# weleen/AGRL.pytorch

Hardware: AMD Instinct MI355X
Metric: frames/sec (fwd+GCN+distmat), MARS seq_len=8 (higher is better)
Workload: dtype fp16; 1 GPU; MARS seq_len=8 bs=32/GPU fp16 fwd+distmat (BASELINE configs[1]): 256x128 frames, VMGN ResNet50x2-branch + 2 graph layers, cosine distmat vs resident 12180 x 4096 gallery; global_batch=32, seq_len=8, gallery_rows_per_gpu=12180, parallelism=dp1, hip_graph=False, ranks=1, devices_visible=1, library=libagrl_hip.so, clip_batches_rotated=3, clip_bytes_rotated=301989888

## Files before the change

### agrl.pytorch_amd/csrc/agrl_common.h

```cpp
#pragma once
#include <hip/hip_runtime.h>
#include <math.h>
#include <stdint.h>
#include <stdio.h>
#include <stdarg.h>

#include "../../include/agrl_hip.h"

#define AGRL_WAVE 64

#ifndef AGRL_LP_F16
#define AGRL_LP_F16 1
#endif
constexpr bool kLpF16 = AGRL_LP_F16 != 0;
typedef unsigned short lp16_t;
typedef __attribute__((ext_vector_type(8))) __bf16 bf16x8_t;
typedef __attribute__((ext_vector_type(8))) _Float16 f16x8_t;
typedef __attribute__((ext_vector_type(4))) float f32x4_t;

void agrl_set_error(const char* fmt, ...);

#define AGRL_CHECK_ARG(cond, ...)       \
    do {                                \
        if (!(cond)) {                  \
            agrl_set_error(__VA_ARGS__); \
            return 1;                   \
        }                               \
    } while (0)

#define AGRL_CHECK_LAUNCH(name)                                                   \
    do {                                                                          \
        hipError_t e__ = hipGetLastError();                                       \
        if (e__ != hipSuccess) {                                                  \
            agrl_set_error("%s: launch failed: %s", name, hipGetErrorString(e__)); \
            return 2;                                                             \
        }                                                                         \
    } while (0)

static inline bool agrl_is_pow2(float v) {
    int e = 0;
    return v > 0.f && v <= 3.4e38f && frexpf(v, &e) == 0.5f;
}
#define AGRL_CHECK_POW2(value, who, name) \
    AGRL_CHECK_ARG(agrl_is_pow2(value), "%s: %s=%g is not a positive finite power of two", who, name, (double)(value))

__attribute__((visibility("hidden"))) int agrl_cu_count();

typedef __attribute__((address_space(3))) void lds_void_t;
typedef __attribute__((address_space(1))) const void gbl_void_t;

__host__ __device__ inline float lp16_to_f32(lp16_t v) {
    if constexpr (kLpF16) {
        return (float)__builtin_bit_cast(_Float16, v);
    } else {
        return __builtin_bit_cast(float, ((uint32_t)v) << 16);
    }
}

__host__ __device__ inline lp16_t f32_to_lp16(float f) {
    if constexpr (kLpF16) {
        return __builtin_bit_cast(unsigned short, (_Float16)f);
    } else {
#if defined(__HIP_DEVICE_COMPILE__)
        const __bf16 h = (__bf16)f;
        return __builtin_bit_cast(unsigned short, h);
#else
        uint32_t u = __builtin_bit_cast(uint32_t, f);
        if ((u & 0x7fffffffu) > 0x7f800000u) return (lp16_t)((u >> 16) | 0x40);
        u += 0x7fffu + ((u >> 16) & 1u);
        return (lp16_t)(u >> 16);
#endif
    }
}

__device__ inline uint32_t pack_lp16x2(float lo, float hi) {
    if constexpr (kLpF16) {
        typedef __attribute__((ext_vector_type(2))) _Float16 f16x2_t;
        const f16x2_t v = {(_Float16)lo, (_Float16)hi};
        return __builtin_bit_cast(uint32_t, v);
    } else {
        typedef __attribute__((ext_vector_type(2))) __bf16 bf16x2_t;
        const bf16x2_t v = {(__bf16)lo, (__bf16)hi};
        return __builtin_bit_cast(uint32_t, v);
    }
}

__device__ inline uint32_t pack_bf16x2(float lo, float hi) {
    typedef __attribute__((ext_vector_type(2))) __bf16 bf16x2_t;
    const bf16x2_t v = {(__bf16)lo, (__bf16)hi};
    return __builtin_bit_cast(uint32_t, v);
}

__device__ inline void unpack_lp16x2(uint32_t w, float& lo, float& hi) {
    if constexpr (kLpF16) {
        typedef __attribute__((ext_vector_type(2))) _Float16 f16x2_t;
        const f16x2_t v = __builtin_bit_cast(f16x2_t, w);
        lo = (float)v[0];
        hi = (float)v[1];
    } else {
        lo = __uint_as_float(w << 16);
        hi = __uint_as_float(w & 0xffff0000u);
    }
}

template <typename TA, typename TB>
__device__ inline __attribute__((ext_vector_type(4))) float mfma_lp16_16x16x32(const TA& a, const TB& b, __attribute__((ext_vector_type(4))) float c) {
    static_assert(sizeof(TA) == 16 && sizeof(TB) == 16, "16-byte MFMA operands");
    if constexpr (kLpF16) {
        return __builtin_amdgcn_mfma_f32_16x16x32_f16(__builtin_bit_cast(f16x8_t, a), __builtin_bit_cast(f16x8_t, b), c, 0, 0, 0);
    } else {
        return __builtin_amdgcn_mfma_f32_16x16x32_bf16(__builtin_bit_cast(bf16x8_t, a), __builtin_bit_cast(bf16x8_t, b), c, 0, 0, 0);
    }
}

__device__ inline float relu_nan(float v) { return __builtin_elementwise_maximum(v, 0.f); }

__device__ inline float wave_sum(float v) {
#pragma unroll
    for (int off = 32; off > 0; off >>= 1) v += __shfl_xor(v, off, 64);
    return v;
}

__device__ inline float wave_max(float v) {
#pragma unroll
    for (int off = 32; off > 0; off >>= 1) v = fmaxf(v, __shfl_xor(v, off, 64));
    return v;
}

__device__ inline int wave_sum_i(int v) {
#pragma unroll
    for (int off = 32; off > 0; off >>= 1) v += __shfl_xor(v, off, 64);
    return v;
}

template <typename T>
struct DT;
template <>
struct DT<float> {
    static constexpr int code = AGRL_F32;
    static constexpr int epc = 4;
    __device__ static inline float ld(const float* p) { return *p; }
    __device__ static inline void st(float* p, float v) { *p = v; }
};
struct f32s_t {
    float v;
};
template <>
struct DT<f32s_t> {
    static constexpr int code = AGRL_F32X3;
    static constexpr int epc = 4;
};
struct f32h_t {
    float v;
};
template <>
struct DT<f32h_t> {
    static constexpr int code = AGRL_F32H3;
    static constexpr int epc = 4;
};
template <>
struct DT<lp16_t> {
    static constexpr int code = AGRL_LP16;
    static constexpr int epc = 8;
    __device__ static inline float ld(const lp16_t* p) { return lp16_to_f32(*p); }
    __device__ static inline void st(lp16_t* p, float v) { *p = f32_to_lp16(v); }
};

static inline int cdiv(int a, int b) { return (a + b - 1) / b; }

#define AGRL_OPT_UNSET (-2147483647 - 1)
struct AgrlOpts {
    int igemm_wide;
    int pool_persist;
    int conv3x3_wide, conv3x3_c64;
    int distmat_tiled;
    int topk_radix;
    int graph_linear_mmajor;
    int conv3x3_n128;
    int conv3x3_fat_pb;
    int conv3x3_half, conv3x3_half_stagger;
    int stem_split_lds;
    int stem_xcd_map;
    int distmat_tile_n;
    int split16_ns;
    int duo_persist;
    int igemm_dbg, conv3x3_dbg;
};
const AgrlOpts& agrl_opts();
inline bool agrl_opt_set(int v) { return v != AGRL_OPT_UNSET; }

#ifdef AGRL_ABLATE
#define AGRL_DBG_BITS(p) ((p).dbg)
#else
#define AGRL_DBG_BITS(p) 0
#endif
```

### agrl.pytorch_amd/csrc/common.hip

```cpp
#include "agrl_common.h"

static thread_local char g_err[512] = "";

void agrl_set_error(const char* fmt, ...) {
    va_list ap;
    va_start(ap, fmt);
    vsnprintf(g_err, sizeof(g_err), fmt, ap);
    va_end(ap);
}

extern "C" int agrl_version(void) { return 100; }
extern "C" const char* agrl_last_error(void) { return g_err; }

extern "C" int agrl_lp16_is_f16(void) { return kLpF16 ? 1 : 0; }

#include <atomic>

int agrl_cu_count() {
    constexpr int kMaxDev = 64;
    static std::atomic<int> cache[kMaxDev];
    int dev = 0;
    if (hipGetDevice(&dev) != hipSuccess) return 256;
    const bool slot = dev >= 0 && dev < kMaxDev;
    int n = slot ? cache[dev].load(std::memory_order_relaxed) : 0;
    if (n > 0) return n;
    if (hipDeviceGetAttribute(&n, hipDeviceAttributeMultiprocessorCount, dev) != hipSuccess || n <= 0) n = 256;
    if (slot) cache[dev].store(n, std::memory_order_relaxed);
    return n;
}

#include <stdlib.h>

static int opt_int(const char* name) {
    const char* e = getenv(name);
    return e ? atoi(e) : AGRL_OPT_UNSET;
}
static int opt_flag(const char* name) {
    const char* e = getenv(name);
    return e && !(e[0] == '0' && e[1] == 0) ? 1 : 0;
}
static AgrlOpts load_opts() {
    AgrlOpts o;
    o.igemm_wide = opt_int("AGRL_IGEMM_WIDE");
    o.pool_persist = opt_flag("AGRL_POOL_PERSIST");
    o.conv3x3_wide = opt_int("AGRL_CONV3X3_WIDE");
    o.conv3x3_c64 = opt_int("AGRL_CONV3X3_C64");
    o.distmat_tiled = opt_flag("AGRL_DISTMAT_TILED");
    o.topk_radix = opt_flag("AGRL_TOPK_RADIX");
    o.graph_linear_mmajor = opt_flag("AGRL_GRAPH_LINEAR_MMAJOR");
    o.conv3x3_n128 = opt_flag("AGRL_CONV3X3_N128");
    o.distmat_tile_n = opt_int("AGRL_DISTMAT_TILE_N");
    o.duo_persist = opt_int("AGRL_DUO_PERSIST");
    o.split16_ns = opt_int("AGRL_SPLIT16_NS");
    o.stem_xcd_map = opt_int("AGRL_STEM_XCD_MAP");
    o.stem_split_lds = opt_int("AGRL_STEM_SPLIT_LDS");
    o.conv3x3_fat_pb = opt_int("AGRL_CONV3X3_FAT_PB");
    o.conv3x3_half = opt_int("AGRL_CONV3X3_HALF");
    o.conv3x3_half_stagger = opt_int("AGRL_CONV3X3_HALF_STAGGER");
#ifdef AGRL_ABLATE
    o.igemm_dbg = agrl_opt_set(opt_int("AGRL_IGEMM_DBG")) ? opt_int("AGRL_IGEMM_DBG") : 0;
    o.conv3x3_dbg = agrl_opt_set(opt_int("AGRL_CONV3X3_DBG")) ? opt_int("AGRL_CONV3X3_DBG") : 0;
#else
    o.igemm_dbg = 0;
    o.conv3x3_dbg = 0;
#endif
    return o;
}
static AgrlOpts g_opts = load_opts();

const AgrlOpts& agrl_opts() { return g_opts; }
extern "C" int agrl_reload_options(void) {
    g_opts = load_opts();
    return 0;
}
extern "C" int agrl_built_with_ablation(void) {
#ifdef AGRL_ABLATE
    return 1;
#else
    return 0;
#endif
}
```

### agrl.pytorch_amd/csrc/stem_dev.h

```cpp
#pragma once
#include "agrl_common.h"
#include "frames_u8.h"

struct StemShape {
    int CH, CW;
    int PH, PW;
    int tiles_h, tiles_w;
    int grid;
};

static inline int stem_shape(const char* who, int N, int H, int W, int pt_h, int pt_w, StemShape* s) {
    AGRL_CHECK_ARG(N > 0 && H >= 7 && W >= 7, "%s: bad shape N=%d H=%d W=%d", who, N, H, W);
    s->CH = (H + 6 - 7) / 2 + 1, s->CW = (W + 6 - 7) / 2 + 1;
    s->PH = (s->CH + 2 - 3) / 2 + 1, s->PW = (s->CW + 2 - 3) / 2 + 1;
    s->tiles_h = cdiv(s->PH, pt_h), s->tiles_w = cdiv(s->PW, pt_w);
    const long long grid = (long long)N * s->tiles_h * s->tiles_w;
    AGRL_CHECK_ARG(grid < (1ll << 31), "%s: grid too large", who);
    s->grid = (int)grid;
    return 0;
}

namespace stem8 {
constexpr int PT = 8;
constexpr int CT = 2 * PT + 1;
constexpr int NPOS = CT * CT;
constexpr int NFRAG = (NPOS + 15) / 16;
constexpr int NWV = 8;
constexpr int NTH = 64 * NWV;
constexpr int FPW = (NFRAG + NWV - 1) / NWV;
constexpr int IT = 2 * (CT - 1) + 7;
constexpr int PWP = 40;
constexpr int PATCH_BYTES = IT * PWP * 8;
constexpr int NPASS = (IT * PWP + NTH - 1) / NTH;
constexpr int WROW_BYTES = 480;
constexpr int W_BYTES = 64 * WROW_BYTES;

struct Tile {
    int n, ph0, pw0, cr0, cc0;
};
__device__ __forceinline__ Tile tile_at(int T, int tiles_w, int tiles_hw) {
    Tile t;
    t.n = T / tiles_hw;
    const int trem = T - t.n * tiles_hw;
    t.ph0 = (trem / tiles_w) * PT, t.pw0 = (trem % tiles_w) * PT;
    t.cr0 = 2 * t.ph0 - 1, t.cc0 = 2 * t.pw0 - 1;
    return t;
}

template <typename TIN, typename... EX>
struct PatchPrefetch {
    static constexpr bool U8 = sizeof...(EX) != 0;
    uint32_t pb[U8 ? NPASS : 1][3];
    float pv[NPASS][3];

    __device__ __forceinline__ void load(const TIN* __restrict__ x, int H, int W, const Tile& t, EX... ex) {
        const int iy0 = 2 * t.cr0 - 3, ix0 = 2 * t.cc0 - 3;
        const TIN* xn = x + (size_t)t.n * 3 * H * W;
        int td = threadIdx.x;
        asm volatile("" : "+v"(td));
#pragma unroll
        for (int i = 0; i < NPASS; ++i) {
            const int e = td + NTH * i;
            const int py = e / PWP, px = e - py * PWP;
            const int iy = iy0 + py, ix = ix0 + px;
            if constexpr (U8) {
                const FramesU8 u8 = frames_u8_of(ex...);
                pb[i][0] = pb[i][1] = pb[i][2] = FRAMES_U8_PAD;
                if (e < IT * PWP && px < IT && (unsigned)iy < (unsigned)H && (unsigned)ix < (unsigned)W) {
                    const uint32_t o = (uint32_t)(iy * W + ix) * u8.pixel_stride;
                    pb[i][0] = xn[o];
                    pb[i][1] = xn[o + (uint32_t)u8.channel_stride];
                    pb[i][2] = xn[o + 2 * (uint32_t)u8.channel_stride];
                }
            } else {
                pv[i][0] = pv[i][1] = pv[i][2] = 0.f;
                if (e < IT * PWP && px < IT && (unsigned)iy < (unsigned)H && (unsigned)ix < (unsigned)W) {
                    const size_t o = (size_t)iy * W + ix;
                    pv[i][0] = xn[o];
                    pv[i][1] = xn[(size_t)H * W + o];
                    pv[i][2] = xn[2 * (size_t)H * W + o];
                }
            }
        }
    }
    __device__ __forceinline__ void normalize(EX... ex) {
        if constexpr (U8) {
            const FramesU8 u8 = frames_u8_of(ex...);
#pragma unroll
            for (int i = 0; i < NPASS; ++i)
#pragma unroll
                for (int c = 0; c < 3; ++c) pv[i][c] = u8.table[c * FRAMES_U8_ROW + pb[i][c]];
        }
    }
};

__device__ __forceinline__ void patch_frag_offsets(int wave, int frow, int g, int (&a_off)[FPW]) {
#pragma unroll
    for (int i = 0; i < FPW; ++i) {
        int pos = (wave + NWV * i) * 16 + frow;
        pos = pos < NPOS ? pos : NPOS - 1;
        const int cy = pos / CT, cx = pos - cy * CT;
        a_off[i] = ((2 * cy) * PWP + 2 * cx + 2 * g) * 8;
    }
}

__device__ __forceinline__ int ct_row(int pos) { return (pos & ~3) | ((pos & 1) << 1) | ((pos >> 1) & 1); }

__device__ __forceinline__ void weights_to_lds(const unsigned char* __restrict__ wpk, unsigned char* s_w, int wave, int lane) {
    for (int piece = wave; piece < W_BYTES / 1024; piece += NWV)
        __builtin_amdgcn_global_load_lds((gbl_void_t*)(wpk + piece * 1024 + lane * 16), (lds_void_t*)(s_w + piece * 1024), 16, 0, 0);
}
}
```

### agrl.pytorch_amd/csrc/stem_mfma.hip

```cpp
#include <stdlib.h>

#include "stem_dev.h"

namespace {
using namespace stem8;

constexpr int CT_BYTES = (NPOS + 3) * 128;
constexpr int REGION_BYTES = CT_BYTES > PATCH_BYTES ? CT_BYTES : PATCH_BYTES;

template <bool SPLIT, typename TIN, typename... EX>
__global__ __launch_bounds__(NTH, 4) void stem_mfma_kernel(const TIN* __restrict__ x, const unsigned char* __restrict__ wpk,
                                                        const float* __restrict__ bias, lp16_t* __restrict__ out, int H,
                                                        int W, int CH, int CW, int PH, int PW, int tiles_w, int tiles_hw,
                                                        int ntiles, int xcd_map, EX... ex) {
    constexpr int TILES_BYTES = SPLIT ? PATCH_BYTES + CT_BYTES : REGION_BYTES;
    __shared__ __attribute__((aligned(16))) unsigned char smem[TILES_BYTES + W_BYTES + 256];
    unsigned char* s_patch = smem;
    unsigned char* s_ct = SPLIT ? smem + PATCH_BYTES : smem;
    unsigned char* s_w = smem + TILES_BYTES;
    float* s_bias = reinterpret_cast<float*>(smem + TILES_BYTES + W_BYTES);

    const int tid = threadIdx.x;
    const int lane = tid & 63;
    const int wave = __builtin_amdgcn_readfirstlane(tid >> 6);
    const int G = gridDim.x;

    weights_to_lds(wpk, s_w, wave, lane);
    if (tid < 64) s_bias[tid] = bias[tid];
    PatchPrefetch<TIN, EX...> pre;
    constexpr bool U8 = decltype(pre)::U8;
    const int frow = lane & 15, g = lane >> 4;
    int a_off[FPW];
    patch_frag_offsets(wave, frow, g, a_off);

    const int nframes = ntiles / tiles_hw;
    const bool xmap = xcd_map && (G & 7) == 0 && nframes >= 8;
    const int xcd = blockIdx.x & 7;
    const int qstep = xmap ? (G >> 3) : G;
    const int qlimit = xmap ? ((nframes - xcd + 7) >> 3) * tiles_hw : ntiles;
    auto tile_of = [&](int q) {
        if (!xmap) return q;
        const int fl = q / tiles_hw;
        return (xcd + 8 * fl) * tiles_hw + (q - fl * tiles_hw);
    };
    int q = xmap ? (int)(blockIdx.x >> 3) : (int)blockIdx.x;
    if (q < qlimit) {
        pre.load(x, H, W, tile_at(tile_of(q), tiles_w, tiles_hw), ex...);
        pre.normalize(ex...);
    }
    for (; q < qlimit; q += qstep) {
        const Tile t = tile_at(tile_of(q), tiles_w, tiles_hw);
        const int n = t.n, ph0 = t.ph0, pw0 = t.pw0, cr0 = t.cr0, cc0 = t.cc0;
        int tw = tid;
        if constexpr (U8) asm volatile("" : "+v"(tw));
#pragma unroll
        for (int i = 0; i < NPASS; ++i) {
            const int e = tw + NTH * i;
            if (e < IT * PWP) {
                uint2 u;
                u.x = pack_lp16x2(pre.pv[i][0], pre.pv[i][1]);
                u.y = (uint32_t)f32_to_lp16(pre.pv[i][2]);
                *reinterpret_cast<uint2*>(s_patch + e * 8) = u;
            }
        }
        asm volatile("s_waitcnt vmcnt(0)" ::: "memory");
        __syncthreads();
        if (q + qstep < qlimit) pre.load(x, H, W, tile_at(tile_of(q + qstep), tiles_w, tiles_hw), ex...);

        f32x4_t acc[FPW][4];
#pragma unroll
        for (int i = 0; i < FPW; ++i)
#pragma unroll
            for (int a = 0; a < 4; ++a) acc[i][a] = f32x4_t{0.f, 0.f, 0.f, 0.f};
#pragma unroll
        for (int r = 0; r < 7; ++r) {
            uint4 wf[4], xf[FPW];
#pragma unroll
            for (int a = 0; a < 4; ++a)
                wf[a] = *reinterpret_cast<const uint4*>(s_w + (a * 16 + frow) * WROW_BYTES + r * 64 + g * 16);
#pragma unroll
            for (int i = 0; i < FPW; ++i) xf[i] = *reinterpret_cast<const uint4*>(s_patch + a_off[i] + r * (PWP * 8));
#pragma unroll
            for (int i = 0; i < FPW; ++i)
#pragma unroll
                for (int a = 0; a < 4; ++a)
                    acc[i][a] = mfma_lp16_16x16x32(wf[a], xf[i], acc[i][a]);
        }
        if constexpr (!SPLIT) __syncthreads();
        int fr = frow, gg = g, tq = tid;
        asm volatile("" : "+v"(fr), "+v"(gg), "+v"(tq));

        const bool interior = cr0 >= 0 && cc0 >= 0 && cr0 + CT <= CH && cc0 + CT <= CW;
        int rowo[FPW], swz[FPW];
        bool live[FPW], in[FPW];
#pragma unroll
        for (int i = 0; i < FPW; ++i) {
            const int pos = (wave + NWV * i) * 16 + fr;
            const int cy = pos / CT, cx = pos - cy * CT;
            live[i] = pos < NPOS;
            in[i] = interior || ((unsigned)(cr0 + cy) < (unsigned)CH && (unsigned)(cc0 + cx) < (unsigned)CW);
            rowo[i] = ct_row(pos) * 128;
            swz[i] = pos & 7;
        }
#pragma unroll
        for (int a = 0; a < 4; ++a) {
            const int ch = a * 16 + gg * 4;
            const float4 bv = *reinterpret_cast<const float4*>(s_bias + ch);
#pragma unroll
            for (int i = 0; i < FPW; ++i) {
                if (live[i]) {
                    const float v0 = relu_nan(acc[i][a][0] + bv.x), v1 = relu_nan(acc[i][a][1] + bv.y);
                    const float v2 = relu_nan(acc[i][a][2] + bv.z), v3 = relu_nan(acc[i][a][3] + bv.w);
                    uint2 u;
                    u.x = pack_lp16x2(v0, v1);
                    u.y = pack_lp16x2(v2, v3);
                    if (!in[i]) u = make_uint2(0u, 0u);
                    *reinterpret_cast<uint2*>(s_ct + rowo[i] + (((ch >> 3) ^ swz[i]) << 4) + ((ch & 4) << 1)) = u;
                }
            }
        }
        __syncthreads();
        if (q + qstep < qlimit) pre.normalize(ex...);

        {
            typedef unsigned short u16x2_t __attribute__((ext_vector_type(2)));
            const int cq = tq & 7;
            const int pp = tq >> 3;
            const int py = pp / PT, px = pp - py * PT;
            const int ph = ph0 + py, pw = pw0 + px;
            if (ph < PH && pw < PW) {
                u16x2_t m[4] = {u16x2_t{0, 0}, u16x2_t{0, 0}, u16x2_t{0, 0}, u16x2_t{0, 0}};
#pragma unroll
                for (int dy = 0; dy < 3; ++dy)
#pragma unroll
                    for (int dx = 0; dx < 3; ++dx) {
                        const int pos = (2 * py + dy) * CT + 2 * px + dx;
                        const uint4 u = *reinterpret_cast<const uint4*>(s_ct + ct_row(pos) * 128 + ((cq ^ (pos & 7)) << 4));
                        const uint32_t w4[4] = {u.x, u.y, u.z, u.w};
#pragma unroll
                        for (int e = 0; e < 4; ++e) m[e] = __builtin_elementwise_max(m[e], __builtin_bit_cast(u16x2_t, w4[e]));
                    }
                const uint4 o = make_uint4(__builtin_bit_cast(uint32_t, m[0]), __builtin_bit_cast(uint32_t, m[1]),
                                           __builtin_bit_cast(uint32_t, m[2]), __builtin_bit_cast(uint32_t, m[3]));
                *reinterpret_cast<uint4*>(out + (((size_t)n * PH + ph) * PW + pw) * 64 + cq * 8) = o;
            }
        }
        if constexpr (!SPLIT) __syncthreads();
    }
}
}

template <typename TIN, typename... EX>
static int launch_stem_mfma(const char* who, const TIN* x, const void* w_packed, const float* bias, void* out, int N, int H, int W,
                            agrl_stream_t stream, EX... ex) {
    AGRL_CHECK_ARG(x && w_packed && bias && out, "%s: null pointer", who);
    StemShape s;
    if (stem_shape(who, N, H, W, PT, PT, &s)) return 1;
    AGRL_CHECK_ARG((((uintptr_t)w_packed) & 15) == 0 && (((uintptr_t)bias) & 15) == 0 && (((uintptr_t)out) & 15) == 0,
                   "%s: misaligned pointer", who);
    const int wgs = 512;
    const unsigned launch = (unsigned)(s.grid < wgs ? s.grid : wgs);
    if (agrl_opts().stem_split_lds != 0)
        hipLaunchKernelGGL((stem_mfma_kernel<true, TIN, EX...>), dim3(launch), dim3(NTH), 0, (hipStream_t)stream, x,
                       (const unsigned char*)w_packed, bias, (lp16_t*)out, H, W, s.CH, s.CW, s.PH, s.PW, s.tiles_w, s.tiles_h * s.tiles_w,
                       s.grid, agrl_opts().stem_xcd_map != 0, ex...);
    else
        hipLaunchKernelGGL((stem_mfma_kernel<false, TIN, EX...>), dim3(launch), dim3(NTH), 0, (hipStream_t)stream, x,
                       (const unsigned char*)w_packed, bias, (lp16_t*)out, H, W, s.CH, s.CW, s.PH, s.PW, s.tiles_w, s.tiles_h * s.tiles_w,
                       s.grid, agrl_opts().stem_xcd_map != 0, ex...);
    AGRL_CHECK_LAUNCH(who);
    return 0;
}

extern "C" int agrl_stem_conv_bn_relu_maxpool_lp16(const float* x, const void* w_packed, const float* bias, void* out,
                                                   int N, int H, int W, agrl_stream_t stream) {
    return launch_stem_mfma("agrl_stem_lp16", x, w_packed, bias, out, N, H, W, stream);
}

extern "C" int agrl_stem_conv_bn_relu_maxpool_lp16_u8(const unsigned char* x, const float* table, int layout, const void* w_packed,
                                                      const float* bias, void* out, int N, int H, int W, agrl_stream_t stream) {
    FramesU8 u8;
    if (frames_u8_args("agrl_stem_lp16_u8", table, layout, H, W, &u8)) return 1;
    return launch_stem_mfma("agrl_stem_lp16_u8", x, w_packed, bias, out, N, H, W, stream, u8);
}
```

Baseline: 71700 frames/s.

## Add register-resident maxpool stem kernel tiling full-width row strips

Adds a new stem conv+BN+ReLU+maxpool kernel that tiles each frame into full-width strips of 8 pooled rows. The 3x3/2 max pool is computed in registers using DPP lane shifts, with small LDS edge buffers and a row carry, instead of writing the conv tile to LDS and re-reading it for pooling. The new kernel is the default when the pooled width fits in 17..32 (the 256x128 input gives 32). The aim is to remove the LDS conv-tile round trip and its barrier and to cut halo recompute. In exchange it adds register pressure and edge-case logic for the boundaries.

```diff
diff --git a/agrl.pytorch_amd/csrc/agrl_common.h b/agrl.pytorch_amd/csrc/agrl_common.h
--- a/agrl.pytorch_amd/csrc/agrl_common.h
+++ b/agrl.pytorch_amd/csrc/agrl_common.h
@@ -181,6 +181,7 @@
     int conv3x3_half, conv3x3_half_stagger;
     int stem_split_lds;
     int stem_xcd_map;
+    int stem_regpool;
     int distmat_tile_n;
     int split16_ns;
     int duo_persist;
diff --git a/agrl.pytorch_amd/csrc/common.hip b/agrl.pytorch_amd/csrc/common.hip
--- a/agrl.pytorch_amd/csrc/common.hip
+++ b/agrl.pytorch_amd/csrc/common.hip
@@ -54,6 +54,7 @@
     o.split16_ns = opt_int("AGRL_SPLIT16_NS");
     o.stem_xcd_map = opt_int("AGRL_STEM_XCD_MAP");
     o.stem_split_lds = opt_int("AGRL_STEM_SPLIT_LDS");
+    o.stem_regpool = opt_int("AGRL_STEM_REGPOOL");
     o.conv3x3_fat_pb = opt_int("AGRL_CONV3X3_FAT_PB");
     o.conv3x3_half = opt_int("AGRL_CONV3X3_HALF");
     o.conv3x3_half_stagger = opt_int("AGRL_CONV3X3_HALF_STAGGER");
diff --git a/agrl.pytorch_amd/csrc/stem_dev.h b/agrl.pytorch_amd/csrc/stem_dev.h
--- a/agrl.pytorch_amd/csrc/stem_dev.h
+++ b/agrl.pytorch_amd/csrc/stem_dev.h
@@ -47,9 +47,11 @@
     return t;
 }
 
-template <typename TIN, typename... EX>
-struct PatchPrefetch {
+template <int IT_, int PWP_, int PWV_, int NTH_, typename TIN, typename... EX>
+struct PatchPrefetchT {
     static constexpr bool U8 = sizeof...(EX) != 0;
+    static constexpr int IT = IT_, PWP = PWP_, NTH = NTH_;
+    static constexpr int NPASS = (IT_ * PWP_ + NTH_ - 1) / NTH_;
     uint32_t pb[U8 ? NPASS : 1][3];
     float pv[NPASS][3];
 
@@ -66,7 +68,7 @@
             if constexpr (U8) {
                 const FramesU8 u8 = frames_u8_of(ex...);
                 pb[i][0] = pb[i][1] = pb[i][2] = FRAMES_U8_PAD;
-                if (e < IT * PWP && px < IT && (unsigned)iy < (unsigned)H && (unsigned)ix < (unsigned)W) {
+                if (e < IT * PWP && px < PWV_ && (unsigned)iy < (unsigned)H && (unsigned)ix < (unsigned)W) {
                     const uint32_t o = (uint32_t)(iy * W + ix) * u8.pixel_stride;
                     pb[i][0] = xn[o];
                     pb[i][1] = xn[o + (uint32_t)u8.channel_stride];
@@ -74,7 +76,7 @@
                 }
             } else {
                 pv[i][0] = pv[i][1] = pv[i][2] = 0.f;
-                if (e < IT * PWP && px < IT && (unsigned)iy < (unsigned)H && (unsigned)ix < (unsigned)W) {
+                if (e < IT * PWP && px < PWV_ && (unsigned)iy < (unsigned)H && (unsigned)ix < (unsigned)W) {
                     const size_t o = (size_t)iy * W + ix;
                     pv[i][0] = xn[o];
                     pv[i][1] = xn[(size_t)H * W + o];
@@ -93,6 +95,8 @@
         }
     }
 };
+template <typename TIN, typename... EX>
+using PatchPrefetch = PatchPrefetchT<IT, PWP, IT, NTH, TIN, EX...>;
 
 __device__ __forceinline__ void patch_frag_offsets(int wave, int frow, int g, int (&a_off)[FPW]) {
 #pragma unroll
@@ -106,8 +110,35 @@
 
 __device__ __forceinline__ int ct_row(int pos) { return (pos & ~3) | ((pos & 1) << 1) | ((pos >> 1) & 1); }
 
-__device__ __forceinline__ void weights_to_lds(const unsigned char* __restrict__ wpk, unsigned char* s_w, int wave, int lane) {
-    for (int piece = wave; piece < W_BYTES / 1024; piece += NWV)
+__device__ __forceinline__ void weights_to_lds(const unsigned char* __restrict__ wpk, unsigned char* s_w, int wave, int lane,
+                                               int nwv = NWV) {
+    for (int piece = wave; piece < W_BYTES / 1024; piece += nwv)
         __builtin_amdgcn_global_load_lds((gbl_void_t*)(wpk + piece * 1024 + lane * 16), (lds_void_t*)(s_w + piece * 1024), 16, 0, 0);
 }
 }
+
+namespace stem_rp {
+constexpr int RT = 8;
+constexpr int NWV = 4;
+constexpr int NTH = 64 * NWV;
+constexpr int RPW = RT / NWV;
+constexpr int NG = 2;
+constexpr int MAX_PW = 16 * NG;
+constexpr int MIN_PW = 16 * (NG - 1) + 1;
+constexpr int IT = 4 * RT + 7;
+constexpr int PWP = 4 * MAX_PW + 6;
+constexpr int ROW_BYTES = PWP * 8;
+constexpr int PATCH_BYTES = IT * ROW_BYTES;
+constexpr int EDGE_BYTES = NWV * (2 * RPW + 1) * 256;
+static_assert(RPW == 2 && NG == 2 && RT % NWV == 0 && ROW_BYTES % 16 == 0, "stem_rp geometry (the kernel's strip walk is written for 2 x 2)");
+
+__device__ __forceinline__ stem8::Tile tile_at(int T, int tiles_h) {
+    stem8::Tile t;
+    t.n = T / tiles_h;
+    t.ph0 = (T - t.n * tiles_h) * RT, t.pw0 = 0;
+    t.cr0 = 2 * t.ph0 - 1, t.cc0 = 0;
+    return t;
+}
+template <typename TIN, typename... EX>
+using PatchPrefetch = stem8::PatchPrefetchT<IT, PWP, PWP, NTH, TIN, EX...>;
+}
diff --git a/agrl.pytorch_amd/csrc/stem_mfma.hip b/agrl.pytorch_amd/csrc/stem_mfma.hip
--- a/agrl.pytorch_amd/csrc/stem_mfma.hip
+++ b/agrl.pytorch_amd/csrc/stem_mfma.hip
@@ -1,4 +1,6 @@
 #include <stdlib.h>
+
+#include <type_traits>
 
 #include "stem_dev.h"
 
@@ -148,7 +150,195 @@
         if constexpr (!SPLIT) __syncthreads();
     }
 }
-}
+
+namespace rp = stem_rp;
+
+__device__ __forceinline__ float fmax_nan(float a, float b) { return __builtin_elementwise_maximum(a, b); }
+template <int CTRL>
+__device__ __forceinline__ float dpp_mov(float old, float src) {
+    return __builtin_bit_cast(float, __builtin_amdgcn_update_dpp(__builtin_bit_cast(int, old), __builtin_bit_cast(int, src), CTRL, 0xf,
+                                                                  0xf, false));
+}
+constexpr int DPP_ROW_SHR1 = 0x111;
+
+template <int NR>
+__device__ __forceinline__ void rp_sweep(const unsigned char* xb, const unsigned char* wb, f32x4_t (&acc)[NR][2][4]) {
+#pragma unroll
+    for (int i = 0; i < NR; ++i)
+#pragma unroll
+        for (int p = 0; p < 2; ++p)
+#pragma unroll
+            for (int a = 0; a < 4; ++a) acc[i][p][a] = f32x4_t{0.f, 0.f, 0.f, 0.f};
+    uint4 wf[2][4], xf[2][NR][2];
+    auto fetch = [&](int r, uint4 (&w)[4], uint4 (&xx)[NR][2]) {
+#pragma unroll
+        for (int a = 0; a < 4; ++a) w[a] = *reinterpret_cast<const uint4*>(wb + a * 16 * WROW_BYTES + r * 64);
+#pragma unroll
+        for (int i = 0; i < NR; ++i)
+#pragma unroll
+            for (int p = 0; p < 2; ++p) xx[i][p] = *reinterpret_cast<const uint4*>(xb + (2 * i + r) * rp::ROW_BYTES + p * 16);
+    };
+    fetch(0, wf[0], xf[0]);
+#pragma unroll
+    for (int r = 0; r < 7; ++r) {
+        if (r < 6) fetch(r + 1, wf[(r + 1) & 1], xf[(r + 1) & 1]);
+#pragma unroll
+        for (int i = 0; i < NR; ++i)
+#pragma unroll
+            for (int p = 0; p < 2; ++p)
+#pragma unroll
+                for (int a = 0; a < 4; ++a) acc[i][p][a] = mfma_lp16_16x16x32(wf[r & 1][a], xf[r & 1][i][p], acc[i][p][a]);
+        __builtin_amdgcn_sched_barrier(0);
+    }
+}
+
+template <int GQ>
+__device__ __forceinline__ void rp_row_max(const f32x4_t (&even)[4], f32x4_t (&odd)[4], float* edge, int frow, bool odd_all_in,
+                                           bool odd_in, f32x4_t (&h)[4]) {
+    if (!odd_all_in) {
+#pragma unroll
+        for (int a = 0; a < 4; ++a)
+#pragma unroll
+            for (int j = 0; j < 4; ++j) odd[a][j] = odd_in ? odd[a][j] : -INFINITY;
+    }
+    f32x4_t first[4];
+    if constexpr (GQ == 0) {
+        if (frow == 15) {
+#pragma unroll
+            for (int a = 0; a < 4; ++a) *reinterpret_cast<f32x4_t*>(edge + 4 * a) = odd[a];
+        }
+#pragma unroll
+        for (int a = 0; a < 4; ++a) first[a] = f32x4_t{-INFINITY, -INFINITY, -INFINITY, -INFINITY};
+    } else {
+#pragma unroll
+        for (int a = 0; a < 4; ++a) first[a] = *reinterpret_cast<const f32x4_t*>(edge + 4 * a);
+    }
+#pragma unroll
+    for (int a = 0; a < 4; ++a)
+#pragma unroll
+        for (int j = 0; j < 4; ++j)
+            h[a][j] = fmax_nan(fmax_nan(even[a][j], odd[a][j]), dpp_mov<DPP_ROW_SHR1>(first[a][j], odd[a][j]));
+}
+
+template <typename TIN, typename... EX>
+__global__ __launch_bounds__(rp::NTH, 2) void stem_regpool_kernel(const TIN* __restrict__ x, const unsigned char* __restrict__ wpk,
+                                                                   const float* __restrict__ bias, lp16_t* __restrict__ out, int H,
+                                                                   int W, int CH, int CW, int PH, int PW, int tiles_h, int ntiles,
+                                                                   int xcd_map, EX... ex) {
+    __shared__ __attribute__((aligned(16))) unsigned char smem[rp::PATCH_BYTES + W_BYTES + 256 + rp::EDGE_BYTES];
+    unsigned char* s_patch = smem;
+    unsigned char* s_w = smem + rp::PATCH_BYTES;
+    float* s_bias = reinterpret_cast<float*>(smem + rp::PATCH_BYTES + W_BYTES);
+
+    const int tid = threadIdx.x;
+    const int lane = tid & 63;
+    const int wave = __builtin_amdgcn_readfirstlane(tid >> 6);
+    const int G = gridDim.x;
+
+    weights_to_lds(wpk, s_w, wave, lane, rp::NWV);
+    if (tid < 64) s_bias[tid] = bias[tid];
+    rp::PatchPrefetch<TIN, EX...> pre;
+    constexpr int NPASS_RP = decltype(pre)::NPASS;
+    const int frow = lane & 15, g = lane >> 4;
+    const unsigned char* xlane = s_patch + 8 * wave * rp::ROW_BYTES + (4 * frow + 2 * g) * 8;
+    const unsigned char* wlane = s_w + frow * WROW_BYTES + g * 16;
+    float* s_edge = reinterpret_cast<float*>(smem + rp::PATCH_BYTES + W_BYTES + 256) + (wave * (2 * rp::RPW + 1) * 4 + g) * 16;
+
+    const int nframes = ntiles / tiles_h;
+    const bool xmap = xcd_map && (G & 7) == 0 && nframes >= 8;
+    const int xcd = blockIdx.x & 7;
+    const int qstep = xmap ? (G >> 3) : G;
+    const int qlimit = xmap ? ((nframes - xcd + 7) >> 3) * tiles_h : ntiles;
+    auto tile_of = [&](int q) {
+        if (!xmap) return q;
+        const int fl = q / tiles_h;
+        return (xcd + 8 * fl) * tiles_h + (q - fl * tiles_h);
+    };
+    int q = xmap ? (int)(blockIdx.x >> 3) : (int)blockIdx.x;
+    if (q < qlimit) pre.load(x, H, W, rp::tile_at(tile_of(q), tiles_h), ex...);
+    for (; q < qlimit; q += qstep) {
+        const Tile t = rp::tile_at(tile_of(q), tiles_h);
+        pre.normalize(ex...);
+        int tw = tid;
+        asm volatile("" : "+v"(tw));
+#pragma unroll
+        for (int i = 0; i < NPASS_RP; ++i) {
+            const int e = tw + rp::NTH * i;
+            if ((i + 1) * rp::NTH <= rp::IT * rp::PWP || e < rp::IT * rp::PWP) {
+                uint2 u;
+                u.x = pack_lp16x2(pre.pv[i][0], pre.pv[i][1]);
+                u.y = (uint32_t)f32_to_lp16(pre.pv[i][2]);
+                *reinterpret_cast<uint2*>(s_patch + e * 8) = u;
+            }
+        }
+        asm volatile("s_waitcnt vmcnt(0)" ::: "memory");
+        __syncthreads();
+        if (q + qstep < qlimit) pre.load(x, H, W, rp::tile_at(tile_of(q + qstep), tiles_h), ex...);
+
+        const int ph_w = t.ph0 + rp::RPW * wave;
+        if (ph_w < PH) {
+            const bool odd_all_in = CW >= 4 * rp::MAX_PW;
+            auto group = [&](auto gq_c) {
+                constexpr int GQ = decltype(gq_c)::value;
+                const unsigned char* xg = xlane + GQ * 512;
+                const int px = 16 * GQ + frow;
+                const bool odd_in = 2 * px + 1 < CW;
+                f32x4_t carry[4];
+                {
+                    f32x4_t acc[1][2][4];
+                    rp_sweep<1>(xg, wlane, acc);
+                    rp_row_max<GQ>(acc[0][0], acc[0][1], s_edge, frow, odd_all_in, odd_in, carry);
+                    if (ph_w == 0) {
+#pragma unroll
+                        for (int a = 0; a < 4; ++a) carry[a] = f32x4_t{-INFINITY, -INFINITY, -INFINITY, -INFINITY};
+                    }
+                }
+#pragma unroll
+                for (int sp = 0; sp < rp::RPW; ++sp) {
+                    const int ph = ph_w + sp;
+                    if (ph < PH) {
+                        f32x4_t acc[2][2][4], ha[4], hb[4];
+                        rp_sweep<2>(xg + (4 * sp + 2) * rp::ROW_BYTES, wlane, acc);
+                        rp_row_max<GQ>(acc[0][0], acc[0][1], s_edge + (2 * sp + 1) * 64, frow, odd_all_in, odd_in, ha);
+                        rp_row_max<GQ>(acc[1][0], acc[1][1], s_edge + (2 * sp + 2) * 64, frow, odd_all_in, odd_in, hb);
+                        if (2 * ph + 1 >= CH) {
+#pragma unroll
+                            for (int a = 0; a < 4; ++a) hb[a] = f32x4_t{-INFINITY, -INFINITY, -INFINITY, -INFINITY};
+                        }
+                        uint32_t pk[4][2];
+#pragma unroll
+                        for (int a = 0; a < 4; ++a) {
+                            const float4 bv = *reinterpret_cast<const float4*>(s_bias + a * 16 + g * 4);
+                            float v[4];
+#pragma unroll
+                            for (int j = 0; j < 4; ++j) v[j] = fmax_nan(fmax_nan(carry[a][j], ha[a][j]), hb[a][j]);
+                            carry[a] = hb[a];
+                            pk[a][0] = pack_lp16x2(relu_nan(v[0] + bv.x), relu_nan(v[1] + bv.y));
+                            pk[a][1] = pack_lp16x2(relu_nan(v[2] + bv.z), relu_nan(v[3] + bv.w));
+                        }
+#pragma unroll
+                        for (int k = 0; k < 2; ++k) {
+                            typedef unsigned int u32x2_t __attribute__((ext_vector_type(2)));
+                            const u32x2_t s0 = __builtin_amdgcn_permlane16_swap(pk[2 * k][0], pk[2 * k + 1][0], false, false);
+                            const u32x2_t s1 = __builtin_amdgcn_permlane16_swap(pk[2 * k][1], pk[2 * k + 1][1], false, false);
+                            if (px < PW) {
+                                const int ch = (2 * k + (g & 1)) * 16 + (g >> 1) * 8;
+                                *reinterpret_cast<uint4*>(out + (((size_t)t.n * PH + ph) * PW + px) * 64 + ch) =
+                                    make_uint4(s0[0], s1[0], s0[1], s1[1]);
+                            }
+                        }
+                    }
+                }
+            };
+            group(std::integral_constant<int, 0>{});
+            group(std::integral_constant<int, 1>{});
+        }
+        __syncthreads();
+    }
+}
+}
+
+constexpr bool STEM_REGPOOL_DEFAULT = true;
 
 template <typename TIN, typename... EX>
 static int launch_stem_mfma(const char* who, const TIN* x, const void* w_packed, const float* bias, void* out, int N, int H, int W,
@@ -158,6 +348,17 @@
     if (stem_shape(who, N, H, W, PT, PT, &s)) return 1;
     AGRL_CHECK_ARG((((uintptr_t)w_packed) & 15) == 0 && (((uintptr_t)bias) & 15) == 0 && (((uintptr_t)out) & 15) == 0,
                    "%s: misaligned pointer", who);
+    const int regpool = agrl_opts().stem_regpool;
+    if ((agrl_opt_set(regpool) ? regpool != 0 : STEM_REGPOOL_DEFAULT) && s.PW >= stem_rp::MIN_PW && s.PW <= stem_rp::MAX_PW) {
+        StemShape r;
+        if (stem_shape(who, N, H, W, stem_rp::RT, stem_rp::MAX_PW, &r)) return 1;
+        const unsigned launch_rp = (unsigned)(r.grid < 512 ? r.grid : 512);
+        hipLaunchKernelGGL((stem_regpool_kernel<TIN, EX...>), dim3(launch_rp), dim3(stem_rp::NTH), 0, (hipStream_t)stream, x,
+                           (const unsigned char*)w_packed, bias, (lp16_t*)out, H, W, r.CH, r.CW, r.PH, r.PW, r.tiles_h, r.grid,
+                           agrl_opts().stem_xcd_map != 0, ex...);
+        AGRL_CHECK_LAUNCH(who);
+        return 0;
+    }
     const int wgs = 512;
     const unsigned launch = (unsigned)(s.grid < wgs ? s.grid : wgs);
     if (agrl_opts().stem_split_lds != 0)
```

Result: faster. 72520 frames/s (median of 6 runs) (+1.1%).
